# yuki-ominato/FER-ViT

Hardware: AMD Instinct MI355X
Metric: training images/sec at 1/2/4/8 MI355X, ViT-B/16 bs=256; fwd+bwd step ms (higher is better)
Workload: dtype bf16; 1 GPU; image_vit ViT-B/16, 224x224 RGB AffectNet-shaped synthetic, bs=256/GPU, train step (fwd+bwd+AdamW), dropout 0.1, CE label_smoothing 0.1; per_gpu_batch=256, global_batch=256, parallelism=dp1

## Files before the change

fer-vit_amd/csrc/attention.hip:

```cpp
#include <stdlib.h>

#include <type_traits>

#include "common.h"
#include "fervit_internal.h"

namespace fer {

constexpr float LOG2E = 1.4426950408889634f;
constexpr float LN2 = 0.6931471805599453f;

FER_DEV int swz(int r) { return (((r >> 1) & 1) << 2) | ((r >> 2) & 3); }
FER_DEV int img_off(int r, int c) { return r * 128 + ((c ^ swz(r)) << 4); }

template <int NB>
FER_DEV void load_image(char* img, const bf16* src, long ld, int N, int dh) {
  for (int idx = threadIdx.x; idx < NB * 32 * 8; idx += blockDim.x) {
    const int r = idx >> 3, c = idx & 7;
    bf16x8 v = {};
    if (r < N && c * 8 < dh) v = *(const bf16x8*)(src + (long)r * ld + c * 8);
    *(bf16x8*)(img + img_off(r, c)) = v;
  }
}

// ... 282 lines not shown
    bar_lds();
    if (wq.q) un = __builtin_amdgcn_readfirstlane(hand[2]);
#pragma unroll 1
    for (int k = 0;; ++k) {
#ifdef FER_ATTN_STAMPS
      const bool st_on = blockIdx.x == 0 && (k == 2 || k == 3);
      const int sb = (k - 2) * 32;
#endif
      AST(sb + 0);
      int unn = -1;
      uint32_t craw = 0;
      if (wq.q) {
        if (claimer && un >= 0) craw = wq_claim_issue(wq.q);
      } else if (un >= 0 && un + (int)gridDim.x < BH) {
        unn = un + gridDim.x;
      }
      if (un >= 0) fwd_dma_unit<NB>(lds + ((k + 1) & 1) * 2 * IMG, rs, un, ldq, N, H, dh, lane);
      AST(sb + 1);
      wait_vm<0>();
      AST(sb + 2);
      asm volatile("" : "+v"(craw));
      if (wq.q && claimer && un >= 0) unn = wq_claim_finish(craw, wq.base, BH);
      if (claimer) hand[k & 1] = unn;
      bar_lds();
      AST(sb + 21);
      u = un;
      un = __builtin_amdgcn_readfirstlane(hand[k & 1]);
      if (u < 0) break;
    }
    return;
  }
  bf16x8 qf[4];
  load_q(qf, u);
  asm volatile("" : "+v"(qf[0]), "+v"(qf[1]), "+v"(qf[2]), "+v"(qf[3]));
  bar_lds();
  if (wq.q) un = __builtin_amdgcn_readfirstlane(hand[2]);
#pragma unroll 1
  for (int k = 0;; ++k) {
#ifdef FER_ATTN_STAMPS
    const bool st_on = blockIdx.x == 0 && (k == 2 || k == 3);
    const int sb = (k - 2) * 32;
#endif
    AST(sb + 0);
    {
      const char* Ki = lds + (k & 1) * 2 * IMG;
      const char* Vi = Ki + IMG;
      const int bh = u, b = u / H, h = u - b * H;
      const uint32_t row = drop_row(bh, N, q);
      float m = -INFINITY, l = 0.f;
      f32x16 ot[2] = {f32x16{}, f32x16{}};
      bf16x8 kfr[4];
#pragma unroll
      for (int s = 0; s < 4; ++s) kfr[s] = rd_row(Ki, lane & 31, 2 * s + hh);
      auto block = [&](int kb, f32x16& st, const bf16x8 (&vfr)[2][2]) {
        if (kb == NB - 1 && NB * 32 > N) {
#pragma unroll
          for (int r = 0; r < 16; ++r)
            if (kb * 32 + acc_row(r, hh) >= N) st[r] = -INFINITY;
        }
        float bm = fmaxf(fmaxf(st[0], st[1]), st[2]);
#pragma unroll
        for (int r = 3; r < 15; r += 2) bm = fmaxf(fmaxf(bm, st[r]), st[r + 1]);
        bm = fmaxf(bm, st[15]);
        bm = xhalf_max(bm) * sl2;
        if (__builtin_amdgcn_ballot_w64(bm > m + 8.f)) {
          const float mn = fmaxf(m, bm);
          const float al = ex2(m - mn);
          m = mn;
          l *= al;
          ot[0] *= al;
          ot[1] *= al;
        }
#pragma unroll
        for (int r = 0; r < 16; ++r) st[r] = ex2(fmaf(st[r], sl2, -m));
        float ls[4];
#pragma unroll
        for (int c = 0; c < 4; ++c) ls[c] = (st[c] + st[c + 4]) + (st[c + 8] + st[c + 12]);
        l += (ls[0] + ls[1]) + (ls[2] + ls[3]);
        if (thr) {
          const uint32_t p0 = (row >> 1) + kb * 16 + 2 * hh;
          uint64_t bal[16];
#pragma unroll
          for (int r = 0; r < 16; r += 2) {
            const uint32_t hv = fer_hash(seed, p0 + (uint32_t)(acc_row(r, 0) >> 1));
            const bool k0 = (hv & 0xFFFFu) >= thr, k1 = (hv >> 16) >= thr;
            st[r] = k0 ? st[r] : 0.f;
            st[r + 1] = k1 ? st[r + 1] : 0.f;
            bal[r] = __builtin_amdgcn_ballot_w64(k0);
            bal[r + 1] = __builtin_amdgcn_ballot_w64(k1);
          }
          if (mask) {
            const uint32_t word = wl_keys8<0>(0u, bal) | wl_keys8<8>(0u, bal + 8);
            __builtin_amdgcn_raw_buffer_store_b32(
                word, rmk, mk_off, __builtin_amdgcn_readfirstlane((int)((((long)bh * NB + kb) * NB + w) * 128)), 0);
          }
        }
#pragma unroll
        for (int s2 = 0; s2 < 2; ++s2) {
          const bf16x8 pf = pack8(st, s2);
#pragma unroll
          for (int db = 0; db < 2; ++db) ot[db] = mfma32(vfr[s2][db], pf, ot[db]);
        }
      };
#pragma unroll 1
      for (int kb = 0; kb < NB; ++kb) {
        bf16x8 vfr[2][2];
#pragma unroll
        for (int s2 = 0; s2 < 2; ++s2)
#pragma unroll
          for (int db = 0; db < 2; ++db) vfr[s2][db] = rd_tr(Vi, kb * 32 + 16 * s2, db * 32, lane);
        f32x16 st = {};
#pragma unroll
        for (int s = 0; s < 4; ++s) st = mfma32(kfr[s], qf[s], st);
        if (kb + 1 < NB) {
#pragma unroll
          for (int s = 0; s < 4; ++s) kfr[s] = rd_row(Ki, (kb + 1) * 32 + (lane & 31), 2 * s + hh);
        }
        AST(sb + 1 + 2 * kb);
        block(kb, st, vfr);
        AST(sb + 2 + 2 * kb);
      }
      load_q(qf, un >= 0 ? un : u);
      l = xhalf_sum(l);
      {
        const float mul = dscale / l;
        const int so = __builtin_amdgcn_readfirstlane((int)((((long)b * N) * ldo + h * dh) * 2));
        auto pack4 = [&](int i) {
          const f32x16& a = ot[i >> 2];
          const int g4 = i & 3;
          const bf16x4 v = {(bf16)(a[4 * g4] * mul), (bf16)(a[4 * g4 + 1] * mul), (bf16)(a[4 * g4 + 2] * mul),
                            (bf16)(a[4 * g4 + 3] * mul)};
          return __builtin_bit_cast(u32x2, v);
        };
#pragma unroll
        for (int i = 0; i < 8; i += 2) {
          const u32x2 pk[2] = {pack4(i), pack4(i + 1)};
          const auto x = __builtin_amdgcn_permlane32_swap(pk[0][0], pk[1][0], false, false);
          const auto y = __builtin_amdgcn_permlane32_swap(pk[0][1], pk[1][1], false, false);
          __builtin_amdgcn_raw_buffer_store_b128(u32x4{x[0], y[0], x[1], y[1]}, ro, o_off(i + hh, lane & 31), so, 0);
        }
        __builtin_amdgcn_raw_buffer_store_b32(__float_as_uint((m + log2f(l)) * LN2), rl, lse_off,
                                              __builtin_amdgcn_readfirstlane(bh * N * 4), 0);
      }
      AST(sb + 20);
    }
    bar_lds();
    AST(sb + 21);
    u = un;
    un = __builtin_amdgcn_readfirstlane(hand[k & 1]);
    if (u < 0) break;
  }
}

template <int NB>
__global__ __launch_bounds__(64 * NB) __attribute__((amdgpu_waves_per_eu(4))) void attn_fwd_occ(
    const bf16* __restrict__ qkv, long ldq, bf16* __restrict__ out, long ldo, float* __restrict__ lse,
    uint32_t* __restrict__ mask, int N, int H, int dh, float sl2, uint32_t thr, float dscale, uint64_t seed) {
  constexpr int IMG = NB * 32 * 128;
  __shared__ __attribute__((aligned(1024))) char lds[2 * IMG];
  const int lane = threadIdx.x & 63, w = __builtin_amdgcn_readfirstlane(threadIdx.x >> 6), hh = lane >> 5;
  const int bh = blockIdx.x, b = bh / H, h = bh - b * H, D = H * dh;
  const int q = w * 32 + (lane & 31);
  seed = step_seed(seed);
  const u32x4 rs = rsrc4(qkv);
  img_dma_asm<NB>(lds, rs, (long)b * N, ldq, D + h * dh, N, dh, w, lane);
  img_dma_asm<NB>(lds + IMG, rs, (long)b * N, ldq, 2 * D + h * dh, N, dh, w, lane);
  const __amdgpu_buffer_rsrc_t rq = make_rsrc(qkv), ro = make_rsrc(out), rl = make_rsrc(lse),
                               rmk = make_rsrc(mask ? (const void*)mask : (const void*)lse);
  bf16x8 qf[4];
  {
    const int so = __builtin_amdgcn_readfirstlane((int)((((long)b * N) * ldq + h * dh) * 2));
#pragma unroll
    for (int s = 0; s < 4; ++s) {
      const int d0 = 16 * s + 8 * hh;
      const uint32_t off = (((uint32_t)q * (uint32_t)ldq + (uint32_t)d0) * 2u) | ((uint32_t)(q >= N || d0 >= dh) << 31);
      qf[s] = __builtin_bit_cast(bf16x8, __builtin_amdgcn_raw_buffer_load_b128(rq, off, so, 0));
    }
  }
  wait_vm<0>();
  asm volatile("" : "+v"(qf[0]), "+v"(qf[1]), "+v"(qf[2]), "+v"(qf[3]));
  bar_lds();
  const char* Ki = lds;
  const char* Vi = lds + IMG;
  const uint32_t row = drop_row(bh, N, q);
  float m = -INFINITY, l = 0.f;
  f32x16 ot[2] = {f32x16{}, f32x16{}};
  const int krb = row_base(lane);
  bf16x8 kfr[4];
#pragma unroll
  for (int s = 0; s < 4; ++s) kfr[s] = rd_rowb(Ki, krb, s);
  auto kblock = [&](int kb, auto tail) {
    constexpr bool TAIL = decltype(tail)::value;
    constexpr int NR = TAIL ? 4 : 16;
    int kr = krb;
    asm volatile("" : "+v"(kr));
    const int lv = TAIL ? (int)__builtin_amdgcn_mbcnt_hi(~0u, __builtin_amdgcn_mbcnt_lo(~0u, 0u)) : lane;
    bf16x8 vfr[2][2];
#pragma unroll
    for (int s2 = 0; s2 < 2; ++s2)
#pragma unroll
      for (int db = 0; db < 2; ++db) vfr[s2][db] = rd_tr(Vi, kb * 32 + 16 * s2, db * 32, lv);
    f32x16 st = {};
#pragma unroll
    for (int s = 0; s < 4; ++s) st = mfma32(kfr[s], qf[s], st);
    if (!TAIL && kb + 1 < NB) {
#pragma unroll
      for (int s = 0; s < 4; ++s) kfr[s] = rd_rowb(Ki + (kb + 1) * 4096, kr, s);
    }
    if (TAIL || (kb == NB - 1 && NB * 32 > N)) {
#pragma unroll
      for (int r = 0; r < NR; ++r)
        if (kb * 32 + acc_row(r, hh) >= N) st[r] = -INFINITY;
    }
    float bm = fmaxf(fmaxf(st[0], st[1]), st[2]);
#pragma unroll
    for (int r = 3; r < NR - 1; r += 2) bm = fmaxf(fmaxf(bm, st[r]), st[r + 1]);
    bm = fmaxf(bm, st[NR - 1]);
    bm = xhalf_max(bm) * sl2;
    if (__builtin_amdgcn_ballot_w64(bm > m + 8.f)) {
      const float mn = fmaxf(m, bm);
      const float al = ex2(m - mn);
      m = mn;
      l *= al;
      ot[0] *= al;
      ot[1] *= al;
    }
#pragma unroll
    for (int r = 0; r < 16; ++r) st[r] = r < NR ? ex2(fmaf(st[r], sl2, -m)) : 0.f;
    if (TAIL) {
      l += (st[0] + st[1]) + (st[2] + st[3]);
    } else {
      float ls[4];
#pragma unroll
      for (int c = 0; c < 4; ++c) ls[c] = (st[c] + st[c + 4]) + (st[c + 8] + st[c + 12]);
      l += (ls[0] + ls[1]) + (ls[2] + ls[3]);
    }
    if (thr) {
      const uint32_t rw = TAIL ? drop_row(bh, N, w * 32 + (lv & 31)) : row;
      const uint32_t p0 = (rw >> 1) + kb * 16 + 2 * hh;
      uint32_t klo = (uint32_t)seed;
      asm volatile("" : "+v"(klo));
      uint32_t word = 0u;
#pragma unroll
      for (int half = 0; half < (TAIL ? 1 : 2); ++half) {
        uint64_t bal[8];
#pragma unroll
        for (int r = 0; r < 8; r += 2) {
          const int rr = 8 * half + r;
          if (rr >= NR) {
            bal[r] = bal[r + 1] = 0;
            continue;
          }
          uint32_t hlo;
          const uint32_t hx = fer_mix_pre(((p0 + (uint32_t)(acc_row(rr, 0) >> 1)) ^ klo) + (uint32_t)(seed >> 32), hlo);
          const bool k0 = hlo >= thr, k1 = (hx >> 16) >= thr;
          st[rr] = k0 ? st[rr] : 0.f;
          st[rr + 1] = k1 ? st[rr + 1] : 0.f;
          bal[r] = __builtin_amdgcn_ballot_w64(k0);
          bal[r + 1] = __builtin_amdgcn_ballot_w64(k1);
        }
        if (mask) word |= TAIL ? wl_keys4(0u, bal) : half ? wl_keys8<8>(0u, bal) : wl_keys8<0>(0u, bal);
      }
      if (mask) {
        const int ln = (int)__builtin_amdgcn_mbcnt_hi(~0u, __builtin_amdgcn_mbcnt_lo(~0u, 0u));
        const uint32_t mk_off = ln < 32 ? (uint32_t)(ln * 4) : FER_OOB;
        __builtin_amdgcn_raw_buffer_store_b32(word, rmk, mk_off,
                                              __builtin_amdgcn_readfirstlane((int)((((long)bh * NB + kb) * NB + w) * 128)), 0);
      }
    }
#pragma unroll
    for (int s2 = 0; s2 < 2; ++s2) {
      const bf16x8 pf = pack8(st, s2);
#pragma unroll
      for (int db = 0; db < 2; ++db) ot[db] = mfma32(vfr[s2][db], pf, ot[db]);
    }
  };
  const bool tail4 = NB * 32 - N >= 24;
#pragma unroll 1
  for (int kb = 0; kb < NB - (tail4 ? 1 : 0); ++kb) kblock(kb, std::false_type{});
  if (tail4) {
    int kbt = NB - 1;
    asm volatile("" : "+s"(kbt));
    kblock(kbt, std::true_type{});
  }
  l = xhalf_sum(l);
  const float mul = dscale / l;
  const int so = __builtin_amdgcn_readfirstlane((int)((((long)b * N) * ldo + h * dh) * 2));
  auto pack4 = [&](int i) {
    const f32x16& a = ot[i >> 2];
    const int g4 = i & 3;
    const bf16x4 v = {(bf16)(a[4 * g4] * mul), (bf16)(a[4 * g4 + 1] * mul), (bf16)(a[4 * g4 + 2] * mul),
                      (bf16)(a[4 * g4 + 3] * mul)};
    return __builtin_bit_cast(u32x2, v);
  };
  const int le = (int)__builtin_amdgcn_mbcnt_hi(~0u, __builtin_amdgcn_mbcnt_lo(~0u, 0u));
  const int qe = w * 32 + (le & 31), he = le >> 5;
#pragma unroll
  for (int i = 0; i < 8; i += 2) {
    const u32x2 pk[2] = {pack4(i), pack4(i + 1)};
    const auto x = __builtin_amdgcn_permlane32_swap(pk[0][0], pk[1][0], false, false);
    const auto y = __builtin_amdgcn_permlane32_swap(pk[0][1], pk[1][1], false, false);
    const u32x4 c = {x[0], y[0], x[1], y[1]};
    const int d = 8 * (i + he);
    const uint32_t off = (((uint32_t)qe * (uint32_t)ldo + (uint32_t)d) * 2u) | ((uint32_t)(qe >= N || d >= dh) << 31);
    __builtin_amdgcn_raw_buffer_store_b128(c, ro, off, so, 0);
  }
  __builtin_amdgcn_raw_buffer_store_b32(__float_as_uint((m + log2f(l)) * LN2), rl,
                                        (qe < N && he == 0) ? (uint32_t)(qe * 4) : FER_OOB,
                                        __builtin_amdgcn_readfirstlane(bh * N * 4), 0);
}

template <int NB>
constexpr int fused_lds_bytes() {
  return 3 * NB * 32 * 128 + 2 * NB * 2048 + 2 * NB * 32 * 4;
}

FER_DEV int ds_off(int r, int c8) { return r * 64 + ((c8 ^ ((r >> 1) & 7)) << 3); }
FER_DEV bf16x8 rd_tr64(const char* img, int rbase, int lane) {
  const int gg = lane >> 4, i = lane & 15, q = i >> 2, p = i & 3;
  const int R = rbase + 4 * (gg >> 1);
  const int c8 = 4 * (gg & 1) + p;
  const char* a1 = img + ds_off(R + q, c8);
  const char* a2 = img + ds_off(R + 8 + q, c8);
  short4_t t1 = __builtin_amdgcn_ds_read_tr16_b64_v4i16((__attribute__((address_space(3))) short4_t*)a1);
  short4_t t2 = __builtin_amdgcn_ds_read_tr16_b64_v4i16((__attribute__((address_space(3))) short4_t*)a2);
  return cat8(t1, t2);
}

struct TrB {
  int a1, a2;
};
FER_DEV TrB tr_base(int lane) {
  const int gg = lane >> 4, i = lane & 15, q = i >> 2, p = i & 3;
  const int R = 4 * (gg >> 1);
  const int c = (16 * (gg & 1) + 4 * p) >> 3, half = (p & 1) * 8;
  const int r1 = R + q, r2 = R + 8 + q;
// ... 936 lines not shown
      }
#pragma unroll
      for (int s2 = 0; s2 < 2; ++s2) {
        const bf16x8 pf = pack8(pd, s2), df = pack8(st, s2);
#pragma unroll
        for (int hf = 0; hf < DH2; ++hf)
#pragma unroll
          for (int db = 0; db < 2; ++db) {
            dv[2 * hf + db] = mfma32(pf, rd_tr(Oi + hf * GEN_IMG, qb * 32 + 16 * s2, db * 32, lane), dv[2 * hf + db]);
            dk[2 * hf + db] = mfma32(df, rd_tr(Qi + hf * GEN_IMG, qb * 32 + 16 * s2, db * 32, lane), dk[2 * hf + db]);
          }
      }
    }
  }
  __syncthreads();
  constexpr int W = 64 * DH2;
  bf16* stg = (bf16*)(lds + w * (2 * 32 * W * 2));
#pragma unroll
  for (int j = 0; j < 2 * DH2; ++j)
#pragma unroll
    for (int r = 0; r < 16; ++r) {
      const int kr = acc_row(r, hh), d = j * 32 + (lane & 31);
      stg[kr * W + d] = (bf16)(dk[j][r] * scale);
      stg[32 * W + kr * W + d] = (bf16)dv[j][r];
    }
#pragma unroll
  for (int i = 0; i < 8 * DH2; ++i) {
    const int t = i * 64 + lane;
    constexpr int CPR = W / 8;
    const int mat = t / (32 * CPR), kr = (t / CPR) & 31, c = t % CPR;
    const int gk = blockIdx.y * GEN_ROWS + w * 32 + kr;
    if (gk < N && c * 8 < dh)
      *(bf16x8*)(dqkv + ((long)b * N + gk) * lddq + (1 + mat) * D + h * dh + c * 8) =
          *(const bf16x8*)(stg + mat * 32 * W + kr * W + c * 8);
  }
}

__global__ void attn_f32_scores(const float* qkv, long ldq, float* P, int B, int N, int H, int dh, float scale) {
  const long idx = blockIdx.x * 256L + threadIdx.x;
  const long total = (long)B * H * N * N;
  if (idx >= total) return;
  const int k = idx % N, q = (idx / N) % N, bh = idx / ((long)N * N), b = bh / H, h = bh % H, D = H * dh;
  const float* qr = qkv + ((long)b * N + q) * ldq + h * dh;
  const float* kr = qkv + ((long)b * N + k) * ldq + D + h * dh;
  float s = 0.f;
  for (int d = 0; d < dh; ++d) s = fmaf(qr[d], kr[d], s);
  P[idx] = s * scale;
}
__global__ void attn_f32_softmax(float* P, float* lse, long rows, int N) {
  const long r = blockIdx.x * 256L + threadIdx.x;
  if (r >= rows) return;
  float* p = P + r * N;
  float m = -INFINITY;
  for (int k = 0; k < N; ++k) m = fmaxf(m, p[k]);
  float l = 0.f;
  for (int k = 0; k < N; ++k) l += expf(p[k] - m);
  for (int k = 0; k < N; ++k) p[k] = expf(p[k] - m) / l;
  if (lse) lse[r] = m + logf(l);
}
__global__ void attn_f32_pv(const float* P, const float* qkv, long ldq, float* out, long ldo, int B, int N, int H,
                            int dh, uint32_t thr, float dscale, uint64_t seed) {
  seed = step_seed(seed);
  const long idx = blockIdx.x * 256L + threadIdx.x;
  const long total = (long)B * H * N * dh;
  if (idx >= total) return;
  const int d = idx % dh, q = (idx / dh) % N, bh = idx / ((long)dh * N), b = bh / H, h = bh % H, D = H * dh;
  const float* pr = P + ((long)bh * N + q) * N;
  const uint32_t rowidx = drop_row(bh, N, q);
  float s = 0.f;
  for (int k = 0; k < N; ++k) {
    float p = pr[k];
    if (thr) p = drop_keep(seed, rowidx + k, thr) ? p * dscale : 0.f;
    s = fmaf(p, qkv[((long)b * N + k) * ldq + 2 * D + h * dh + d], s);
  }
  out[((long)b * N + q) * ldo + h * dh + d] = s;
}
__global__ void attn_f32_ds(const float* P, float* G, const float* qkv, long ldq, const float* out, long ldo,
                            const float* dout, long lddo, int B, int N, int H, int dh, uint32_t thr, float dscale,
                            uint64_t seed) {
  seed = step_seed(seed);
  const long r = blockIdx.x * 256L + threadIdx.x;
  const long rows = (long)B * H * N;
  if (r >= rows) return;
  const int q = r % N, bh = r / N, b = bh / H, h = bh % H, D = H * dh;
  const float* o = out + ((long)b * N + q) * ldo + h * dh;
  const float* g = dout + ((long)b * N + q) * lddo + h * dh;
  float dd = 0.f;
  for (int d = 0; d < dh; ++d) dd = fmaf(o[d], g[d], dd);
  for (int k = 0; k < N; ++k) {
    const float* v = qkv + ((long)b * N + k) * ldq + 2 * D + h * dh;
    float dp = 0.f;
    for (int d = 0; d < dh; ++d) dp = fmaf(g[d], v[d], dp);
    if (thr) dp = drop_keep(seed, drop_row(bh, N, q) + k, thr) ? dp * dscale : 0.f;
    G[r * N + k] = P[r * N + k] * (dp - dd);
  }
}
__global__ void attn_f32_grads(const float* P, const float* G, const float* qkv, long ldq, const float* dout,
                               long lddo, float* dqkv, long lddq, int B, int N, int H, int dh, float scale,
                               uint32_t thr, float dscale, uint64_t seed) {
  seed = step_seed(seed);
  const long idx = blockIdx.x * 256L + threadIdx.x;
  const long total = (long)B * H * N * dh;
  if (idx >= total) return;
  const int d = idx % dh, t = (idx / dh) % N, bh = idx / ((long)dh * N), b = bh / H, h = bh % H, D = H * dh;
  const long rb = (long)bh * N;
  float dq = 0.f, dk = 0.f, dv = 0.f;
  for (int j = 0; j < N; ++j) {
    dq = fmaf(G[(rb + t) * N + j], qkv[((long)b * N + j) * ldq + D + h * dh + d], dq);
    dk = fmaf(G[(rb + j) * N + t], qkv[((long)b * N + j) * ldq + h * dh + d], dk);
    float p = P[(rb + j) * N + t];
    if (thr) p = drop_keep(seed, drop_row(bh, N, j) + t, thr) ? p * dscale : 0.f;
    dv = fmaf(p, dout[((long)b * N + j) * lddo + h * dh + d], dv);
  }
  float* o = dqkv + ((long)b * N + t) * lddq + h * dh + d;
  o[0] = dq * scale;
  o[D] = dk * scale;
  o[2 * D] = dv;
}

#define FER_NB_SWITCH(NB, ...)     \
  switch (NB) {                    \
    case 1: { constexpr int NB_ = 1; __VA_ARGS__; } break; \
    case 2: { constexpr int NB_ = 2; __VA_ARGS__; } break; \
    case 3: { constexpr int NB_ = 3; __VA_ARGS__; } break; \
    case 4: { constexpr int NB_ = 4; __VA_ARGS__; } break; \
    case 5: { constexpr int NB_ = 5; __VA_ARGS__; } break; \
    case 6: { constexpr int NB_ = 6; __VA_ARGS__; } break; \
    case 7: { constexpr int NB_ = 7; __VA_ARGS__; } break; \
    default: { constexpr int NB_ = 8; __VA_ARGS__; } break; \
  }

}

using namespace fer;

int fer::set_step_ptr_attention(const uint64_t* p) { return set_step_ptr_here(p) == hipSuccess ? 0 : -1; }

#ifdef FER_ATTN_STAMPS
extern "C" int fer_debug_attn_stamps(unsigned long long* host) {
  return hipMemcpyFromSymbol(host, HIP_SYMBOL(g_ast), sizeof(unsigned long long) * 9 * 64) == hipSuccess ? 0 : 1;
}
extern "C" int fer_debug_attn_bwd_stamps(unsigned long long* host) {
  return hipMemcpyFromSymbol(host, HIP_SYMBOL(g_bst), sizeof(unsigned long long) * 8 * 128) == hipSuccess ? 0 : 1;
}
#endif

extern "C" int64_t fer_attention_ws(int dtype, int B, int N, int H) {
  const int64_t cs = std::max<int64_t>(fer_colsum_ws(B * N, 3 * H * 128), (int64_t)B * 7 * 3 * H * 64 * 4);
  return (dtype == FER_F32 ? (int64_t)2 * B * H * N * N * 4 : 0) + cs;
}

static bool pers_path(int dtype, int N, int dh) { return dtype == FER_BF16 && N <= 224 && dh <= 64; }
static int g_fwd_kernel = 0;
static int64_t lse_floats(int B, int N, int H) { return ((int64_t)B * H * N + 63) / 64 * 64; }
static bool fixed_stride() { return fixed_stride_mode(); }
static int n_cus() {
  static const int n = [] {
    int dev = 0, c = 0;
    if (hipGetDevice(&dev) != hipSuccess || hipDeviceGetAttribute(&c, hipDeviceAttributeMultiprocessorCount, dev) != hipSuccess)
      c = 256;
    return c > 0 ? c : 256;
  }();
  return n;
}

template <typename Kern>
static int pers_occ(Kern k, int threads) {
  int n = 0;
  if (hipOccupancyMaxActiveBlocksPerMultiprocessor(&n, k, threads, 0) != hipSuccess || n < 1) n = 1;
  return std::min(n, 8);
}

extern "C" int64_t fer_attention_saved_floats(int dtype, int B, int N, int H, int dh, uint32_t drop_thresh) {
  const int64_t nb = (N + 31) / 32;
  const int64_t mask_words = (drop_thresh && pers_path(dtype, N, dh)) ? (int64_t)B * H * nb * nb * 32 : 0;
  return lse_floats(B, N, H) + mask_words;
}

extern "C" int fer_attention_fwd(int dtype, const void* qkv, int64_t ld_qkv, void* out, int64_t ld_out, float* lse,
                                 int64_t saved_floats, int B, int N, int H, int dh, float scale, uint32_t drop_thresh,
                                 float drop_scale, uint64_t seed, float* ws, int64_t ws_bytes, fer_stream_t stream) {
  if (B <= 0) return 0;
  hipStream_t st = (hipStream_t)stream;
  if (saved_floats < fer_attention_saved_floats(dtype, B, N, H, dh, drop_thresh))
    return set_error("attention_fwd: saved-state buffer smaller than fer_attention_saved_floats()");
  if (dtype == FER_F32) {
    if (!ws || ws_bytes < fer_attention_ws(dtype, B, N, H)) return set_error("attention_fwd: fp32 workspace too small");
    const long pe = (long)B * H * N * N, rows = (long)B * H * N, oe = rows * dh;
    hipLaunchKernelGGL(attn_f32_scores, dim3(ceil_div(pe, 256)), dim3(256), 0, st, (const float*)qkv, (long)ld_qkv, ws,
                       B, N, H, dh, scale);
    hipLaunchKernelGGL(attn_f32_softmax, dim3(ceil_div(rows, 256)), dim3(256), 0, st, ws, lse, rows, N);
    hipLaunchKernelGGL(attn_f32_pv, dim3(ceil_div(oe, 256)), dim3(256), 0, st, (const float*)ws, (const float*)qkv,
                       (long)ld_qkv, (float*)out, (long)ld_out, B, N, H, dh, drop_thresh, drop_scale, seed);
    return hip_check("attention_fwd_f32");
  }
  if (dh > 128 || dh % 8) return set_error("attention_fwd(bf16): needs dh <= 128, dh % 8 == 0");
  if (check_drop_range(drop_thresh, (long)B * H * N * (N + (N & 1)), "attention_fwd: dropout over >= 2^32 probabilities"))
    return -1;
  if (ld_qkv % 8 || ld_out % 4) return set_error("attention_fwd(bf16): misaligned leading dimension");
  if ((long)B * N * ld_qkv * 2 >= 0x7FFFFFF0L || (long)B * N * ld_out * 2 >= 0x7FFFFFF0L)
    return set_error("attention_fwd(bf16): qkv or out exceeds 2 GiB");
  const float sl2 = scale * LOG2E;
  if (N <= 256 && dh <= 64 && N > 224) {
    const int nb = (N + 31) / 32;
    FER_NB_SWITCH(nb, hipLaunchKernelGGL(attn_fwd_bf16<NB_>, dim3(B * H), dim3(64 * NB_), 0, st, (const bf16*)qkv,
                                         (long)ld_qkv, (bf16*)out, (long)ld_out, lse, N, H, dh, sl2, drop_thresh,
                                         drop_scale, seed));
  } else if (N <= 224 && dh <= 64 && (g_fwd_kernel == 2 || (g_fwd_kernel == 0 && drop_thresh && (N + 31) / 32 >= 4))) {
    const int nb = (N + 31) / 32;
    uint32_t* mask = (drop_thresh && pers_path(dtype, N, dh)) ? (uint32_t*)(lse + lse_floats(B, N, H)) : nullptr;
#define FER_FOCC2(NBV)                                                                                     \
  case NBV:                                                                                                \
    hipLaunchKernelGGL((attn_fwd_occ<NBV>), dim3(B * H), dim3(64 * NBV), 0, st, (const bf16*)qkv,          \
                       (long)ld_qkv, (bf16*)out, (long)ld_out, lse, mask, N, H, dh, sl2, drop_thresh,       \
                       drop_scale, seed);                                                                  \
    break;
    switch (nb) {
      FER_FOCC2(1) FER_FOCC2(2) FER_FOCC2(3) FER_FOCC2(4) FER_FOCC2(5) FER_FOCC2(6) FER_FOCC2(7)
    }
#undef FER_FOCC2
  } else if (N <= 224 && dh <= 64) {
    const int nb = (N + 31) / 32;
    uint32_t* mask = (drop_thresh && pers_path(dtype, N, dh)) ? (uint32_t*)(lse + lse_floats(B, N, H)) : nullptr;
    int occ = 1;
#define FER_FOCC(NBV)                                                               \
  case NBV: {                                                                       \
    static const int o = pers_occ(attn_fwd_pers<NBV>, 64 * (NBV + 1));             \
    occ = o;                                                                        \
  } break;
    switch (nb) { FER_FOCC(1) FER_FOCC(2) FER_FOCC(3) FER_FOCC(4) FER_FOCC(5) FER_FOCC(6) FER_FOCC(7) }
#undef FER_FOCC
    const int grid = std::min(B * H, n_cus() * occ);
    const WqArgs wq = fixed_stride() ? WqArgs{} : wq_prepare_here(st, grid, B * H);
#define FER_FPERS(NBV)                                                                                     \
  case NBV:                                                                                                \
    hipLaunchKernelGGL((attn_fwd_pers<NBV>), dim3(grid), dim3(64 * (NBV + 1)), 0, st, (const bf16*)qkv,    \
                       (long)ld_qkv, (bf16*)out, (long)ld_out, lse, mask, B * H, N, H, dh, sl2, drop_thresh, \
                       drop_scale, seed, wq);                                                             \
    break;
    switch (nb) {
      FER_FPERS(1) FER_FPERS(2) FER_FPERS(3) FER_FPERS(4) FER_FPERS(5) FER_FPERS(6) FER_FPERS(7)
    }
#undef FER_FPERS
    wq_check_launch(st, wq);
  } else {
    const dim3 grid(B * H, (N + GEN_ROWS - 1) / GEN_ROWS);
    if (dh <= 64)
      hipLaunchKernelGGL(attn_fwd_gen<1>, grid, dim3(256), 0, st, (const bf16*)qkv, (long)ld_qkv, (bf16*)out,
                         (long)ld_out, lse, N, H, dh, sl2, drop_thresh, drop_scale, seed);
    else
      hipLaunchKernelGGL(attn_fwd_gen<2>, grid, dim3(256), 0, st, (const bf16*)qkv, (long)ld_qkv, (bf16*)out,
                         (long)ld_out, lse, N, H, dh, sl2, drop_thresh, drop_scale, seed);
  }
  return hip_check("attention_fwd_bf16");
}

extern "C" int fer_attention_bwd(int dtype, const void* qkv, int64_t ld_qkv, const void* out, int64_t ld_out,
                                 const void* dout, int64_t ld_dout, const float* lse, int64_t saved_floats, void* dqkv,
                                 int64_t ld_dqkv, float* ws, int64_t ws_bytes, int B, int N, int H, int dh,
                                 float scale, uint32_t drop_thresh, float drop_scale, uint64_t seed, float* colsum,
                                 int colsum_accumulate, fer_stream_t stream) {
  if (B <= 0) return 0;
  hipStream_t st = (hipStream_t)stream;
  if (saved_floats < fer_attention_saved_floats(dtype, B, N, H, dh, drop_thresh))
    return set_error("attention_bwd: saved-state buffer smaller than fer_attention_saved_floats()");
  const int D3 = 3 * H * dh;
  if (colsum && (!ws || ws_bytes < fer_attention_ws(dtype, B, N, H)))
    return set_error("attention_bwd: colsum needs the workspace (fer_attention_ws bytes)");
  auto colsum_pass = [&](float* cws, int64_t cbytes) -> int {
    return fer_colsum(dtype, dqkv, ld_dqkv, B * N, D3, colsum, colsum_accumulate, nullptr, cws, cbytes, stream);
  };
  if (dtype == FER_F32) {
    if (!ws || ws_bytes < fer_attention_ws(dtype, B, N, H)) return set_error("attention_bwd: fp32 workspace too small");
    const long pe = (long)B * H * N * N, rows = (long)B * H * N, oe = rows * dh;
    float* P = ws;
    float* G = ws + pe;
    hipLaunchKernelGGL(attn_f32_scores, dim3(ceil_div(pe, 256)), dim3(256), 0, st, (const float*)qkv, (long)ld_qkv, P,
                       B, N, H, dh, scale);
    hipLaunchKernelGGL(attn_f32_softmax, dim3(ceil_div(rows, 256)), dim3(256), 0, st, P, (float*)nullptr, rows, N);
    hipLaunchKernelGGL(attn_f32_ds, dim3(ceil_div(rows, 256)), dim3(256), 0, st, (const float*)P, G,
                       (const float*)qkv, (long)ld_qkv, (const float*)out, (long)ld_out, (const float*)dout,
                       (long)ld_dout, B, N, H, dh, drop_thresh, drop_scale, seed);
    hipLaunchKernelGGL(attn_f32_grads, dim3(ceil_div(oe, 256)), dim3(256), 0, st, (const float*)P, (const float*)G,
                       (const float*)qkv, (long)ld_qkv, (const float*)dout, (long)ld_dout, (float*)dqkv,
                       (long)ld_dqkv, B, N, H, dh, scale, drop_thresh, drop_scale, seed);
    int rc = hip_check("attention_bwd_f32");
    if (rc || !colsum) return rc;
    return colsum_pass(ws + 2 * pe, ws_bytes - 2 * pe * 4);
  }
  if (dh > 128 || dh % 8) return set_error("attention_bwd(bf16): needs dh <= 128, dh % 8 == 0");
  if (check_drop_range(drop_thresh, (long)B * H * N * (N + (N & 1)), "attention_bwd: dropout over >= 2^32 probabilities"))
    return -1;
  if (ld_qkv % 8 || ld_out % 8 || ld_dout % 8 || ld_dqkv % 8) return set_error("attention_bwd(bf16): misaligned ld");
  if ((long)B * N * ld_qkv * 2 >= 0x7FFFFFF0L || (long)B * N * ld_dout * 2 >= 0x7FFFFFF0L ||
      (long)B * N * ld_dqkv * 2 >= 0x7FFFFFF0L || (long)B * N * ld_out * 2 >= 0x7FFFFFF0L)
    return set_error("attention_bwd(bf16): operand exceeds 2 GiB (buffer-resource range)");
  const int nb = (N + 31) / 32;
  const float sl2 = scale * LOG2E;
  if (pers_path(dtype, N, dh)) {
    const uint32_t* mask = drop_thresh ? (const uint32_t*)(lse + lse_floats(B, N, H)) : nullptr;
    if (colsum) ws = reduction_ws(ws, (size_t)B * nb * D3 * 4, D3, st);
    int occ = 1;
#define FER_BOCC(NBV)                                                               \
  case NBV: {                                                                       \
    static const int o = pers_occ(attn_bwd_pers<NBV>, bwd_threads<NBV>());                   \
    occ = o;                                                                        \
  } break;
    switch (nb) { FER_BOCC(1) FER_BOCC(2) FER_BOCC(3) FER_BOCC(4) FER_BOCC(5) FER_BOCC(6) FER_BOCC(7) }
#undef FER_BOCC
    const int grid = std::min(B * H, n_cus() * occ);
    const WqArgs wq = fixed_stride() ? WqArgs{} : wq_prepare_here(st, grid, B * H);
#define FER_PERS(NBV)                                                                                          \
  case NBV:                                                                                                    \
    hipLaunchKernelGGL(attn_bwd_pers<NBV>, dim3(grid), dim3(bwd_threads<NBV>()), 0, st, (const bf16*)qkv,                \
                       (long)ld_qkv, (const bf16*)out, (long)ld_out, (const bf16*)dout, (long)ld_dout, lse, mask, \
                       (bf16*)dqkv, (long)ld_dqkv, B * H, N, H, dh, scale, sl2, drop_scale, colsum ? ws : nullptr, \
                       wq);                                                                                      \
    break;
    switch (nb) {
      FER_PERS(1) FER_PERS(2) FER_PERS(3) FER_PERS(4) FER_PERS(5) FER_PERS(6) FER_PERS(7)
    }
#undef FER_PERS
    wq_check_launch(st, wq);
    int rc = hip_check("attention_bwd_bf16_pers");
    if (rc || !colsum) return rc;
    part_reduce(ws, B * nb, D3, D3, D3, colsum, nullptr, nullptr, colsum_accumulate, nullptr, st);
    return hip_check("attention_bwd_colsum");
  }
  if (nb <= 8 && dh <= 64) {
    if (colsum) ws = reduction_ws(ws, (size_t)B * D3 * 4, D3, st);
#define FER_FUSED(NBV)                                                                                       \
  case NBV:                                                                                                  \
    hipLaunchKernelGGL(attn_bwd_fused_bf16<NBV>, dim3(B * H), dim3(64 * NBV), 0, st, (const bf16*)qkv,       \
                       (long)ld_qkv, (const bf16*)out, (long)ld_out, (const bf16*)dout, (long)ld_dout, lse,   \
                       (bf16*)dqkv, (long)ld_dqkv, N, H, dh, scale, sl2, drop_thresh, drop_scale, seed,      \
                       colsum ? ws : nullptr);                                                              \
    break;
    switch (nb) {
      FER_FUSED(1) FER_FUSED(2) FER_FUSED(3) FER_FUSED(4) FER_FUSED(5) FER_FUSED(6) FER_FUSED(7)
      FER_FUSED(8)
    }
#undef FER_FUSED
    int rc = hip_check("attention_bwd_bf16_fused");
    if (rc || !colsum) return rc;
    part_reduce(ws, B, D3, D3, D3, colsum, nullptr, nullptr, colsum_accumulate, nullptr, st);
    return hip_check("attention_bwd_colsum");
  }
  const dim3 grid(B * H, (N + GEN_ROWS - 1) / GEN_ROWS);
#define FER_GEN(DH2)                                                                                           \
  hipLaunchKernelGGL(attn_dq_gen<DH2>, grid, dim3(256), 0, st, (const bf16*)qkv, (long)ld_qkv, (const bf16*)out, \
                     (long)ld_out, (const bf16*)dout, (long)ld_dout, lse, (bf16*)dqkv, (long)ld_dqkv, N, H, dh,    \
                     scale, sl2, drop_thresh, drop_scale, seed);                                                \
  hipLaunchKernelGGL(attn_dkv_gen<DH2>, grid, dim3(256), 0, st, (const bf16*)qkv, (long)ld_qkv, (const bf16*)out, \
                     (long)ld_out, (const bf16*)dout, (long)ld_dout, lse, (bf16*)dqkv, (long)ld_dqkv, N, H, dh,     \
                     scale, sl2, drop_thresh, drop_scale, seed);
  if (dh <= 64) {
    FER_GEN(1)
  } else {
    FER_GEN(2)
  }
#undef FER_GEN
  int rc = hip_check("attention_bwd_bf16");
  if (rc || !colsum) return rc;
  return colsum_pass(ws, ws_bytes);
}

extern "C" int fer_attention_set_fwd_kernel(int k) {
  if (k < 0 || k > 2) return fer::set_error("attention_set_fwd_kernel: 0 (default), 1 (persistent) or 2 (occupancy form)");
  g_fwd_kernel = k;
  return 0;
}
```

Measured before the change: 7573 images/s.

## Use a 16-query MFMA tile for the ragged last query block in attention forward

For ViT-B/16 (N=197, dh=64) the last 32-query block holds only 5 valid queries. The occupancy-form forward kernel now gives that last wave a separate 16x16x32 MFMA path that processes 16 queries, with its own online softmax, dropout mask packing and output/LSE stores. The aim is to cut wasted MFMA and exp work on padded query rows. It adds a large new code path, including inline writelane assembly for mask bits, which must reproduce the existing dropout mask layout exactly.

```diff
diff --git a/fer-vit_amd/csrc/attention.hip b/fer-vit_amd/csrc/attention.hip
--- a/fer-vit_amd/csrc/attention.hip
+++ b/fer-vit_amd/csrc/attention.hip
@@ -458,7 +458,151 @@
   }
 }
 
+FER_DEV f32x4 mfma16(bf16x8 a, bf16x8 b, f32x4 c) { return __builtin_amdgcn_mfma_f32_16x16x32_bf16(a, b, c, 0, 0, 0); }
+FER_DEV float x16_max(float v) {
+  const auto r = __builtin_amdgcn_permlane16_swap(__float_as_uint(v), __float_as_uint(v), false, false);
+  return fmaxf(__uint_as_float(r[0]), __uint_as_float(r[1]));
+}
+FER_DEV float x16_sum(float v) {
+  const auto r = __builtin_amdgcn_permlane16_swap(__float_as_uint(v), __float_as_uint(v), false, false);
+  return __uint_as_float(r[0]) + __uint_as_float(r[1]);
+}
+FER_DEV uint32_t wl_tile16(const uint64_t* b) {
+  uint32_t w = 0u;
+  asm volatile(
+      "s_nop 4\n\t"
+      "v_writelane_b32 %0, %1, 0\n\tv_writelane_b32 %0, %2, 16\n\t"
+      "v_writelane_b32 %0, %3, 1\n\tv_writelane_b32 %0, %4, 17\n\t"
+      "v_writelane_b32 %0, %5, 2\n\tv_writelane_b32 %0, %6, 18\n\t"
+      "v_writelane_b32 %0, %7, 3\n\tv_writelane_b32 %0, %8, 19\n\t"
+      "v_writelane_b32 %0, %9, 8\n\tv_writelane_b32 %0, %10, 24\n\t"
+      "v_writelane_b32 %0, %11, 9\n\tv_writelane_b32 %0, %12, 25\n\t"
+      "v_writelane_b32 %0, %13, 10\n\tv_writelane_b32 %0, %14, 26\n\t"
+      "v_writelane_b32 %0, %15, 11\n\tv_writelane_b32 %0, %16, 27"
+      : "+v"(w)
+      : "s"((uint32_t)b[0]), "s"((uint32_t)(b[0] >> 32)), "s"((uint32_t)b[1]), "s"((uint32_t)(b[1] >> 32)),
+        "s"((uint32_t)b[2]), "s"((uint32_t)(b[2] >> 32)), "s"((uint32_t)b[3]), "s"((uint32_t)(b[3] >> 32)),
+        "s"((uint32_t)b[4]), "s"((uint32_t)(b[4] >> 32)), "s"((uint32_t)b[5]), "s"((uint32_t)(b[5] >> 32)),
+        "s"((uint32_t)b[6]), "s"((uint32_t)(b[6] >> 32)), "s"((uint32_t)b[7]), "s"((uint32_t)(b[7] >> 32)));
+  return w;
+}
+
 template <int NB>
+FER_DEV void fwd_tile16(const char* Ki, const char* Vi, const bf16x8 (&qt)[4], int qb, int bh, int b, int h, int N,
+                        int dh, long ldo, __amdgpu_buffer_rsrc_t ro, __amdgpu_buffer_rsrc_t rl,
+                        __amdgpu_buffer_rsrc_t rmk, bool mask, float sl2, uint32_t thr, float dscale, uint64_t seed) {
+  const int ln = (int)__builtin_amdgcn_mbcnt_hi(~0u, __builtin_amdgcn_mbcnt_lo(~0u, 0u));
+  const int i = ln & 15, g = ln >> 4;
+  const int q = qb * 32 + i;
+  const int kbase = 16 * (g >> 1) + 4 * (g & 1);
+  const int kr = 16 * (i >> 3) + 4 * ((i >> 2) & 1) + (i & 3);
+  const int ka0 = img_off(kr, g), ka1 = img_off(kr + 8, g);
+  const int vr = kbase + (i >> 2), vp = i & 3;
+  const int va0 = vr * 128 + (((vp >> 1) ^ swz(vr)) << 4) + (vp & 1) * 8;
+  const int va1 = (vr + 8) * 128 + (((vp >> 1) ^ swz(vr + 8)) << 4) + (vp & 1) * 8;
+  const uint32_t row = drop_row(bh, N, q);
+  float m = -INFINITY, l = 0.f;
+  f32x4 ot[4] = {f32x4{}, f32x4{}, f32x4{}, f32x4{}};
+#pragma unroll 1
+  for (int kb = 0; kb < NB; ++kb) {
+    const char* Kb = Ki + kb * 4096;
+    const char* Vb = Vi + kb * 4096;
+    bf16x8 kf[2][2], vf[4];
+#pragma unroll
+    for (int s = 0; s < 2; ++s) {
+      kf[0][s] = *(const bf16x8*)(Kb + (ka0 ^ (s << 6)));
+      kf[1][s] = *(const bf16x8*)(Kb + (ka1 ^ (s << 6)));
+    }
+#pragma unroll
+    for (int dt = 0; dt < 4; ++dt) {
+      const short4_t t1 = __builtin_amdgcn_ds_read_tr16_b64_v4i16(
+          (__attribute__((address_space(3))) short4_t*)(Vb + (va0 ^ (dt << 5))));
+      const short4_t t2 = __builtin_amdgcn_ds_read_tr16_b64_v4i16(
+          (__attribute__((address_space(3))) short4_t*)(Vb + (va1 ^ (dt << 5))));
+      vf[dt] = cat8(t1, t2);
+    }
+    f32x4 st[2];
+#pragma unroll
+    for (int tt = 0; tt < 2; ++tt) {
+      st[tt] = mfma16(kf[tt][0], qt[0], f32x4{});
+      st[tt] = mfma16(kf[tt][1], qt[1], st[tt]);
+    }
+    if (kb == NB - 1 && NB * 32 > N) {
+#pragma unroll
+      for (int tt = 0; tt < 2; ++tt)
+#pragma unroll
+        for (int j = 0; j < 4; ++j)
+          if (kb * 32 + kbase + 8 * tt + j >= N) st[tt][j] = -INFINITY;
+    }
+    float bm = fmaxf(fmaxf(fmaxf(st[0][0], st[0][1]), fmaxf(st[0][2], st[0][3])),
+                     fmaxf(fmaxf(st[1][0], st[1][1]), fmaxf(st[1][2], st[1][3])));
+    bm = x16_max(xhalf_max(bm)) * sl2;
+    if (__builtin_amdgcn_ballot_w64(bm > m + 8.f)) {
+      const float mn = fmaxf(m, bm);
+      const float al = ex2(m - mn);
+      m = mn;
+      l *= al;
+#pragma unroll
+      for (int dt = 0; dt < 4; ++dt) ot[dt] *= al;
+    }
+#pragma unroll
+    for (int tt = 0; tt < 2; ++tt)
+#pragma unroll
+      for (int j = 0; j < 4; ++j) st[tt][j] = ex2(fmaf(st[tt][j], sl2, -m));
+    {
+      float ls[4];
+#pragma unroll
+      for (int j = 0; j < 4; ++j) ls[j] = xhalf_sum(st[0][j] + st[1][j]);
+      l += (ls[0] + ls[1]) + (ls[2] + ls[3]);
+    }
+    if (thr) {
+      const uint32_t p0 = (row >> 1) + kb * 16 + (uint32_t)(kbase >> 1);
+      uint64_t bal[8];
+#pragma unroll
+      for (int tt = 0; tt < 2; ++tt)
+#pragma unroll
+        for (int j = 0; j < 4; j += 2) {
+          uint32_t hlo;
+          const uint32_t hx = fer_mix_pre(((p0 + (uint32_t)(4 * tt + (j >> 1))) ^ (uint32_t)seed) + (uint32_t)(seed >> 32), hlo);
+          const bool k0 = hlo >= thr, k1 = (hx >> 16) >= thr;
+          st[tt][j] = k0 ? st[tt][j] : 0.f;
+          st[tt][j + 1] = k1 ? st[tt][j + 1] : 0.f;
+          bal[4 * tt + j] = __builtin_amdgcn_ballot_w64(k0);
+          bal[4 * tt + j + 1] = __builtin_amdgcn_ballot_w64(k1);
+        }
+      if (mask) {
+        const uint32_t wd = wl_tile16(bal);
+        const uint32_t sh = __builtin_amdgcn_update_dpp(0u, wd, 0x114, 0xF, 0xF, true);
+        const uint32_t word = (ln & 4) ? (sh >> 16) : (wd & 0xFFFFu);
+        __builtin_amdgcn_raw_buffer_store_b32(word, rmk, ln < 32 ? (uint32_t)(ln * 4) : FER_OOB,
+                                              __builtin_amdgcn_readfirstlane((int)((((long)bh * NB + kb) * NB + qb) * 128)), 0);
+      }
+    }
+    bf16x8 pf;
+#pragma unroll
+    for (int j = 0; j < 4; ++j) {
+      pf[j] = (bf16)st[0][j];
+      pf[4 + j] = (bf16)st[1][j];
+    }
+#pragma unroll
+    for (int dt = 0; dt < 4; ++dt) ot[dt] = mfma16(vf[dt], pf, ot[dt]);
+  }
+  l = x16_sum(l);
+  const float mul = dscale / l;
+  const int so = __builtin_amdgcn_readfirstlane((int)((((long)b * N) * ldo + h * dh) * 2));
+#pragma unroll
+  for (int dt = 0; dt < 4; ++dt) {
+    const int d = 16 * dt + 4 * g;
+    const bf16x4 v = {(bf16)(ot[dt][0] * mul), (bf16)(ot[dt][1] * mul), (bf16)(ot[dt][2] * mul), (bf16)(ot[dt][3] * mul)};
+    const uint32_t off = (((uint32_t)q * (uint32_t)ldo + (uint32_t)d) * 2u) | ((uint32_t)(q >= N || d >= dh) << 31);
+    __builtin_amdgcn_raw_buffer_store_b64(__builtin_bit_cast(u32x2, v), ro, off, so, 0);
+  }
+  __builtin_amdgcn_raw_buffer_store_b32(__float_as_uint((m + log2f(l)) * LN2), rl,
+                                        (q < N && g == 0) ? (uint32_t)(q * 4) : FER_OOB,
+                                        __builtin_amdgcn_readfirstlane(bh * N * 4), 0);
+}
+
+template <int NB, bool T16 = false>
 __global__ __launch_bounds__(64 * NB) __attribute__((amdgpu_waves_per_eu(4))) void attn_fwd_occ(
     const bf16* __restrict__ qkv, long ldq, bf16* __restrict__ out, long ldo, float* __restrict__ lse,
     uint32_t* __restrict__ mask, int N, int H, int dh, float sl2, uint32_t thr, float dscale, uint64_t seed) {
@@ -478,7 +622,9 @@
     const int so = __builtin_amdgcn_readfirstlane((int)((((long)b * N) * ldq + h * dh) * 2));
 #pragma unroll
     for (int s = 0; s < 4; ++s) {
-      const int d0 = 16 * s + 8 * hh;
+      const bool tile = T16 && w == NB - 1;
+      const int q = tile ? (NB - 1) * 32 + (lane & 15) : w * 32 + (lane & 31);
+      const int d0 = tile ? (s < 2 ? 32 * s + 8 * (lane >> 4) : 64) : 16 * s + 8 * hh;
       const uint32_t off = (((uint32_t)q * (uint32_t)ldq + (uint32_t)d0) * 2u) | ((uint32_t)(q >= N || d0 >= dh) << 31);
       qf[s] = __builtin_bit_cast(bf16x8, __builtin_amdgcn_raw_buffer_load_b128(rq, off, so, 0));
     }
@@ -488,6 +634,10 @@
   bar_lds();
   const char* Ki = lds;
   const char* Vi = lds + IMG;
+  if (T16 && w == NB - 1) {
+    fwd_tile16<NB>(Ki, Vi, qf, NB - 1, bh, b, h, N, dh, ldo, ro, rl, rmk, mask != nullptr, sl2, thr, dscale, seed);
+    return;
+  }
   const uint32_t row = drop_row(bh, N, q);
   float m = -INFINITY, l = 0.f;
   f32x16 ot[2] = {f32x16{}, f32x16{}};
@@ -1730,6 +1880,7 @@
 
 static bool pers_path(int dtype, int N, int dh) { return dtype == FER_BF16 && N <= 224 && dh <= 64; }
 static int g_fwd_kernel = 0;
+static bool tile16_shape(int N, int dh) { return dh == 64 && N > 96 && N <= 224 && (N - 1) % 32 < 16; }
 static int64_t lse_floats(int B, int N, int H) { return ((int64_t)B * H * N + 63) / 64 * 64; }
 static bool fixed_stride() { return fixed_stride_mode(); }
 static int n_cus() {
@@ -1784,7 +1935,8 @@
     FER_NB_SWITCH(nb, hipLaunchKernelGGL(attn_fwd_bf16<NB_>, dim3(B * H), dim3(64 * NB_), 0, st, (const bf16*)qkv,
                                          (long)ld_qkv, (bf16*)out, (long)ld_out, lse, N, H, dh, sl2, drop_thresh,
                                          drop_scale, seed));
-  } else if (N <= 224 && dh <= 64 && (g_fwd_kernel == 2 || (g_fwd_kernel == 0 && drop_thresh && (N + 31) / 32 >= 4))) {
+  } else if (N <= 224 && dh <= 64 &&
+             (g_fwd_kernel >= 2 || (g_fwd_kernel == 0 && drop_thresh && (N + 31) / 32 >= 4))) {
     const int nb = (N + 31) / 32;
     uint32_t* mask = (drop_thresh && pers_path(dtype, N, dh)) ? (uint32_t*)(lse + lse_floats(B, N, H)) : nullptr;
 #define FER_FOCC2(NBV)                                                                                     \
@@ -1793,9 +1945,20 @@
                        (long)ld_qkv, (bf16*)out, (long)ld_out, lse, mask, N, H, dh, sl2, drop_thresh,       \
                        drop_scale, seed);                                                                  \
     break;
-    switch (nb) {
-      FER_FOCC2(1) FER_FOCC2(2) FER_FOCC2(3) FER_FOCC2(4) FER_FOCC2(5) FER_FOCC2(6) FER_FOCC2(7)
-    }
+#define FER_FOCC16(NBV)                                                                                    \
+  case NBV:                                                                                                \
+    hipLaunchKernelGGL((attn_fwd_occ<NBV, true>), dim3(B * H), dim3(64 * NBV), 0, st,                      \
+                       (const bf16*)qkv, (long)ld_qkv, (bf16*)out, (long)ld_out, lse, mask, N, H, dh, sl2,   \
+                       drop_thresh, drop_scale, seed);                                                     \
+    break;
+    if (tile16_shape(N, dh) && g_fwd_kernel != 2) {
+      switch (nb) { FER_FOCC16(4) FER_FOCC16(5) FER_FOCC16(6) FER_FOCC16(7) }
+    } else {
+      switch (nb) {
+        FER_FOCC2(1) FER_FOCC2(2) FER_FOCC2(3) FER_FOCC2(4) FER_FOCC2(5) FER_FOCC2(6) FER_FOCC2(7)
+      }
+    }
+#undef FER_FOCC16
 #undef FER_FOCC2
   } else if (N <= 224 && dh <= 64) {
     const int nb = (N + 31) / 32;
@@ -1944,7 +2107,9 @@
 }
 
 extern "C" int fer_attention_set_fwd_kernel(int k) {
-  if (k < 0 || k > 2) return fer::set_error("attention_set_fwd_kernel: 0 (default), 1 (persistent) or 2 (occupancy form)");
+  if (k < 0 || k > 3)
+    return fer::set_error("attention_set_fwd_kernel: 0 (default), 1 (persistent), 2 (occupancy form) or 3 (occupancy "
+                          "form with a 16-query last tile)");
   g_fwd_kernel = k;
   return 0;
 }
```

Result: no change. 7545 images/s (-0.4%).
